# ramanathanlab/distllm

Hardware: NVIDIA H100
Metric: embedded chunks/sec @512-tok (higher is better)
Workload: dtype bf16

## Files before the change

### distllm_b200/csrc/b2e_api.cu

```cuda
#include "../../include/b2e.h"
#include "../../include/b2e_debug.h"

#include <cuda.h>
#include <cuda_runtime.h>

#include <cstdarg>
#include <cstdio>
#include <cstdlib>
#include <cstring>
#include <string>
#include <utility>
#include <vector>

#include "attention.cuh"
#include "binsearch.cuh"
#include "common.cuh"
#include "gemm.cuh"
#include "mistral_ops.cuh"
#include "pack.cuh"
#include "rowops.cuh"
#include "topk.cuh"
#include "topk_tc.cuh"

using namespace b2e;

#ifdef B2E_STORAGE_BF16
#define B2E_TMAP_DTYPE CU_TENSOR_MAP_DATA_TYPE_BFLOAT16
constexpr int kStorageDtype = B2E_DTYPE_BF16;
#else
#define B2E_TMAP_DTYPE CU_TENSOR_MAP_DATA_TYPE_FLOAT16
constexpr int kStorageDtype = B2E_DTYPE_F16;
#endif

namespace {

thread_local std::string g_err;

int fail(int code, const char* fmt, ...) {
  char buf[512];
  va_list ap;
  va_start(ap, fmt);
  vsnprintf(buf, sizeof buf, fmt, ap);
  va_end(ap);
  g_err = buf;
  return code;
}

#define CUDA_TRY(expr)                                                                    \
  do {                                                                                    \
    cudaError_t e_ = (expr);                                                              \
    if (e_ != cudaSuccess)                                                                \
      return fail(B2E_ERR_CUDA, "%s failed: %s (%s:%d)", #expr, cudaGetErrorString(e_),   \
                  __FILE__, __LINE__);                                                    \
  } while (0)

typedef CUresult (*EncodeTiledFn)(CUtensorMap*, CUtensorMapDataType, cuuint32_t, void*,
                                  const cuuint64_t*, const cuuint64_t*, const cuuint32_t*,
                                  const cuuint32_t*, CUtensorMapInterleave, CUtensorMapSwizzle,
                                  CUtensorMapL2promotion, CUtensorMapFloatOOBfill);

EncodeTiledFn get_encode_fn() {
  static EncodeTiledFn fn = nullptr;
  if (fn) return fn;
  void* p = nullptr;
  cudaDriverEntryPointQueryResult q;
  if (cudaGetDriverEntryPoint("cuTensorMapEncodeTiled", &p, cudaEnableDefault, &q) != cudaSuccess ||
      q != cudaDriverEntryPointSuccess)
    return nullptr;
  fn = reinterpret_cast<EncodeTiledFn>(p);
  return fn;
}

int make_tmap_h16(CUtensorMap* tm, const void* base, uint64_t rows, uint64_t cols,
                   uint32_t box_rows, uint32_t box_cols = 64) {
  EncodeTiledFn fn = get_encode_fn();
  if (!fn) return fail(B2E_ERR_CUDA, "cuTensorMapEncodeTiled entry point unavailable");
  cuuint64_t dims[2] = {cols, rows};
  cuuint64_t strides[1] = {cols * 2};
  cuuint32_t box[2] = {box_cols, box_rows};
  cuuint32_t estr[2] = {1, 1};
  CUresult r = fn(tm, B2E_TMAP_DTYPE, 2, const_cast<void*>(base), dims, strides,
                  box, estr, CU_TENSOR_MAP_INTERLEAVE_NONE,
                  box_cols == 64 ? CU_TENSOR_MAP_SWIZZLE_128B : CU_TENSOR_MAP_SWIZZLE_64B,
                  CU_TENSOR_MAP_L2_PROMOTION_L2_256B, CU_TENSOR_MAP_FLOAT_OOB_FILL_NONE);
  if (r != CUDA_SUCCESS)
    return fail(B2E_ERR_CUDA, "cuTensorMapEncodeTiled(rows=%llu, cols=%llu, box_rows=%u) -> %d",
                (unsigned long long)rows, (unsigned long long)cols, box_rows, (int)r);
  return B2E_OK;
}

int make_tmap_f32(CUtensorMap* tm, const void* base, uint64_t rows, uint64_t cols, uint32_t box_rows) {
  EncodeTiledFn fn = get_encode_fn();
  if (!fn) return fail(B2E_ERR_CUDA, "cuTensorMapEncodeTiled entry point unavailable");
  cuuint64_t dims[2] = {cols, rows};
  cuuint64_t strides[1] = {cols * 4};
  cuuint32_t box[2] = {32, box_rows};
  cuuint32_t estr[2] = {1, 1};
  CUresult r = fn(tm, CU_TENSOR_MAP_DATA_TYPE_FLOAT32, 2, const_cast<void*>(base), dims, strides, box, estr,
                  CU_TENSOR_MAP_INTERLEAVE_NONE, CU_TENSOR_MAP_SWIZZLE_128B, CU_TENSOR_MAP_L2_PROMOTION_L2_256B,
                  CU_TENSOR_MAP_FLOAT_OOB_FILL_NONE);
  if (r != CUDA_SUCCESS)
    return fail(B2E_ERR_CUDA, "cuTensorMapEncodeTiled f32(rows=%llu, cols=%llu, box_rows=%u) -> %d",
                (unsigned long long)rows, (unsigned long long)cols, box_rows, (int)r);
  return B2E_OK;
}

struct DeviceInfo {
  int sms = 0;
  int cc_major = 0;
  bool ok = false;
};

int device_info(int device, DeviceInfo* info) {
  int n = 0;
  if (cudaGetDeviceCount(&n) != cudaSuccess || n == 0) {
    cudaGetLastError();
    return fail(B2E_ERR_NO_DEVICE, "no CUDA device visible; libb2e has no CPU fallback");
  }
  if (device < 0 || device >= n) return fail(B2E_ERR_INVALID, "device %d out of range", device);
  cudaDeviceProp p;
  CUDA_TRY(cudaGetDeviceProperties(&p, device));
  if (p.major != 9 || p.minor != 0)
    return fail(B2E_ERR_NO_DEVICE, "device %d is sm_%d%d; libb2e is built for sm_90a only", device,
                p.major, p.minor);
  info->sms = p.multiProcessorCount;
  info->cc_major = p.major;
  info->ok = true;
  return B2E_OK;
}

int current_device_info(DeviceInfo* info) {
  int dev = 0;
  if (cudaGetDevice(&dev) != cudaSuccess) {
    cudaGetLastError();
    return fail(B2E_ERR_NO_DEVICE, "no CUDA device visible; libb2e has no CPU fallback");
  }
  static DeviceInfo cache[64];
  if (dev < 64 && cache[dev].ok) {
    *info = cache[dev];
    return B2E_OK;
  }
  int rc = device_info(dev, info);
  if (rc == B2E_OK && dev < 64) cache[dev] = *info;
  return rc;
}

template <typename Kern>
int ensure_smem_attr(Kern kern, int bytes) {
  static std::vector<std::pair<const void*, int>> done;
  int dev = 0;
  CUDA_TRY(cudaGetDevice(&dev));
  const void* key = reinterpret_cast<const void*>(kern);
  for (const auto& d : done)
    if (d.first == key && d.second == dev) return B2E_OK;
  CUDA_TRY(cudaFuncSetAttribute(kern, cudaFuncAttributeMaxDynamicSharedMemorySize, bytes));
  done.emplace_back(key, dev);
  return B2E_OK;
}

int check_gemm_shape(int M, int N, int K) {
  if (M <= 0 || N <= 0 || K <= 0) return fail(B2E_ERR_INVALID, "gemm: empty shape %dx%dx%d", M, N, K);
  if (N % 128 != 0) return fail(B2E_ERR_INVALID, "gemm: N=%d must be a multiple of 128", N);
  if (K % 64 != 0) return fail(B2E_ERR_INVALID, "gemm: K=%d must be a multiple of 64", K);
  return B2E_OK;
}

bool g_gemm_profiling = false;

template <int EPI>
int launch_gemm_epi(const CUtensorMap& ta, const CUtensorMap& tb, void* out, const float* bias,
                    const h16* resid, int M, int N, int K, cudaStream_t st, const int* m_dev) {
  auto kern = gemm_h16_wgmma_kernel<EPI>;
  if constexpr (EPI == EPI_BIAS)
    if (g_gemm_profiling) kern = gemm_h16_wgmma_kernel<EPI, true>;
  int rc = ensure_smem_attr(kern, GEMM_SMEM_BYTES);
  if (rc) return rc;
  DeviceInfo dev;
  if ((rc = current_device_info(&dev))) return rc;
  const long long tiles = (long long)(N / GEMM_BN) * ((M + GEMM_BM - 1) / GEMM_BM);
  if (tiles > 0x7fffffffLL) return fail(B2E_ERR_INVALID, "gemm: %lld output tiles exceed one grid", tiles);
  CUtensorMap tm_out;
  if ((rc = make_tmap_h16(&tm_out, out, M, epi_is_glu(EPI) ? N / 2 : N, GEMM_BM))) return rc;
  const unsigned grid = (unsigned)(tiles < dev.sms ? tiles : dev.sms);
  kern<<<grid, GEMM_THREADS, GEMM_SMEM_BYTES, st>>>(ta, tb, tm_out, static_cast<h16*>(out), bias, resid, M, N, K,
                                                    m_dev);
  CUDA_TRY(cudaGetLastError());
  return B2E_OK;
}

int launch_gemm(const CUtensorMap& ta, const CUtensorMap& tb, void* out, const float* bias,
                const void* resid, int M, int N, int K, int epi, cudaStream_t st, const int* m_dev = nullptr) {
  const h16* r = static_cast<const h16*>(resid);
  switch (epi) {
    case B2E_EPI_BIAS: return launch_gemm_epi<EPI_BIAS>(ta, tb, out, bias, r, M, N, K, st, m_dev);
    case B2E_EPI_BIAS_GELU: return launch_gemm_epi<EPI_BIAS_GELU>(ta, tb, out, bias, r, M, N, K, st, m_dev);
    case B2E_EPI_BIAS_RESID: return launch_gemm_epi<EPI_BIAS_RESID>(ta, tb, out, bias, r, M, N, K, st, m_dev);
    case B2E_EPI_SWIGLU: return launch_gemm_epi<EPI_SWIGLU>(ta, tb, out, bias, r, M, N, K, st, m_dev);
    case B2E_EPI_GEGLU: return launch_gemm_epi<EPI_GEGLU>(ta, tb, out, bias, r, M, N, K, st, m_dev);
  }
  return fail(B2E_ERR_INVALID, "unknown epilogue %d", epi);
}

struct AttnScratch {
  float* bias = nullptr;
  int* kv_chunks = nullptr;
  int* plain_chunks = nullptr;
  size_t cap_bias = 0, cap_b = 0;
  uint64_t gen = 0;
  int device = -1;
  int ensure(int B, int S_pad) {
    int dev = 0;
    CUDA_TRY(cudaGetDevice(&dev));
    if (dev != device) {
      release();
      device = dev;
      ++gen;
    }
    if ((size_t)B * S_pad > cap_bias || (size_t)B > cap_b) ++gen;
    if ((size_t)B * S_pad > cap_bias) {
      cudaFree(bias);
      bias = nullptr;
      cap_bias = 0;
      CUDA_TRY(cudaMalloc(&bias, sizeof(float) * (size_t)B * S_pad));
      cap_bias = (size_t)B * S_pad;
    }
    if ((size_t)B > cap_b) {
      cudaFree(kv_chunks); cudaFree(plain_chunks);
      kv_chunks = plain_chunks = nullptr;
      cap_b = 0;
      CUDA_TRY(cudaMalloc(&kv_chunks, sizeof(int) * B));
      CUDA_TRY(cudaMalloc(&plain_chunks, sizeof(int) * B));
      cap_b = B;
    }
    return B2E_OK;
  }
  void release() {
    cudaFree(bias); cudaFree(kv_chunks); cudaFree(plain_chunks);
    bias = nullptr; kv_chunks = plain_chunks = nullptr; cap_bias = cap_b = 0;
  }
};

inline int attn_s_pad(int S) { return (S + AT_KC - 1) / AT_KC * AT_KC; }

int attention_prepare(AttnScratch& sc, const int64_t* mask, int B, int S, cudaStream_t st) {
  int rc;
  const int S_pad = attn_s_pad(S);
  if ((rc = sc.ensure(B, S_pad))) return rc;
  attn_prep_kernel<<<(B + 7) / 8, 256, 0, st>>>(mask, sc.bias, sc.kv_chunks, sc.plain_chunks, B, S, S_pad);
  CUDA_TRY(cudaGetLastError());
  return B2E_OK;
}

struct SeqLayout {
  const int* cu = nullptr;
  const int* len = nullptr;
  const int* t_real = nullptr;
  const int* tok_src = nullptr;
};

template <int D, int MODE, int V>
int launch_attention_kernel(const CUtensorMap& tm, const AttnScratch& sc, void* ctx, int B, int S, int heads,
                            int kv_heads, int window, cudaStream_t st, const SeqLayout& lay) {
  using Cfg = AtCfg<D, V>;
  auto kern = attention_kernel<D, MODE, V>;
  int rc = ensure_smem_attr(kern, Cfg::SMEM_BYTES);
  if (rc) return rc;
  CUtensorMap tm_ctx = {};
  if ((V & 128) && (rc = make_tmap_h16(&tm_ctx, ctx, (uint64_t)B * S, (uint64_t)heads * D, 64, Cfg::COLS))) return rc;
  const float scale_log2e = 1.4426950408889634f / sqrtf(static_cast<float>(D));
  const long long ctas = (long long)heads * B * ((S + Cfg::QT - 1) / Cfg::QT);
  if (ctas > 0x7fffffffLL)
    return fail(B2E_ERR_INVALID, "attention: %lld CTAs (heads=%d B=%d S=%d) exceed one grid", ctas, heads, B, S);
  kern<<<(unsigned)ctas, Cfg::THREADS, Cfg::SMEM_BYTES, st>>>(tm, tm_ctx, sc.bias, sc.kv_chunks, sc.plain_chunks, B, S,
                                                    attn_s_pad(S), heads, kv_heads, window, scale_log2e, lay.cu,
                                                    lay.len, static_cast<h16*>(ctx));
  CUDA_TRY(cudaGetLastError());
  return B2E_OK;
}

constexpr int AT_DEFAULT_VARIANT = 193;
int g_att3_variant = -1;
inline int att3_variant() {
  if (g_att3_variant < 0) {
    const char* e = getenv("B2E_ATT3");
    g_att3_variant = e ? atoi(e) : AT_DEFAULT_VARIANT;
  }
  return g_att3_variant;
}

int launch_attention(const CUtensorMap& tkv, const AttnScratch& sc, void* ctx, int B, int S, int heads,
                     cudaStream_t st, int window = 0, const SeqLayout& lay = SeqLayout()) {
  const int v = att3_variant();
#define B2E_ATT(MODE, V) launch_attention_kernel<64, MODE, V>(tkv, sc, ctx, B, S, heads, heads, window, st, lay)
  if (window > 0) {
    switch (v & 192) {
      case 0: return B2E_ATT(1, 0);
      case 64: return B2E_ATT(1, 64);
      case 128: return B2E_ATT(1, 128);
      case 192: return B2E_ATT(1, 192);
    }
    return fail(B2E_ERR_INVALID, "windowed attention: variant %d has no instantiation (bits 6-7 of the variant pick "
                "0, 64, 128 or 192)", v);
  }
  switch (v) {
    case 0: return B2E_ATT(0, 0);
    case 1: return B2E_ATT(0, 1);
    case 5: return B2E_ATT(0, 5);
    case 64: return B2E_ATT(0, 64);
    case 65: return B2E_ATT(0, 65);
    case 69: return B2E_ATT(0, 69);
    case 193: return B2E_ATT(0, 193);
    case 261: return B2E_ATT(0, 261);
    case 321: return B2E_ATT(0, 321);
  }
#undef B2E_ATT
  return fail(B2E_ERR_INVALID, "attention variant %d is not instantiated (0,1,5,64,65,69,193,261,321)", v);
}

int launch_attention_causal_d128(const void* qkv, AttnScratch& sc, void* ctx, int B, int S, int heads,
                                 int kv_heads, int window, cudaStream_t st, const SeqLayout& lay = SeqLayout()) {
  CUtensorMap tm;
  const int rc = make_tmap_h16(&tm, qkv, (uint64_t)B * S, (uint64_t)(heads + 2 * kv_heads) * 128, AT_KC);
  if (rc) return rc;
  return launch_attention_kernel<128, 2, 0>(tm, sc, ctx, B, S, heads, kv_heads, window, st, lay);
}

constexpr int AT_D32_VARIANT = 1;

int launch_attention_bidir(const CUtensorMap& tqkv, const AttnScratch& sc, void* ctx, int B, int S, int heads,
                           int head_dim, cudaStream_t st, const SeqLayout& lay = SeqLayout()) {
  if (head_dim == 32)
    return launch_attention_kernel<32, 0, AT_D32_VARIANT>(tqkv, sc, ctx, B, S, heads, heads, 0, st, lay);
  return launch_attention(tqkv, sc, ctx, B, S, heads, st, 0, lay);
}

#define DISPATCH_H(H, CALL)                                         \
  switch (H) {                                                      \
    case 256: { constexpr int HW = 256; CALL; break; }              \
    case 384: { constexpr int HW = 384; CALL; break; }              \
    case 512: { constexpr int HW = 512; CALL; break; }              \
    case 640: { constexpr int HW = 640; CALL; break; }              \
    case 768: { constexpr int HW = 768; CALL; break; }              \
    case 1024: { constexpr int HW = 1024; CALL; break; }            \
    case 1280: { constexpr int HW = 1280; CALL; break; }            \
    case 2048: { constexpr int HW = 2048; CALL; break; }            \
    case 2560: { constexpr int HW = 2560; CALL; break; }            \
    case 4096: { constexpr int HW = 4096; CALL; break; }            \
    default: return fail(B2E_ERR_INVALID, "hidden size %d not supported (need 256*{1,2,3,4,5,8,10,16}, 384 or 640)", (H)); \
  }

inline int row_blocks(int rows) { return (rows + ROW_WARPS - 1) / ROW_WARPS; }

int check_h(int H) {
  if (H == 384 || H == 640) return B2E_OK;
  if (H % 256 != 0) return fail(B2E_ERR_INVALID, "hidden size %d must be a multiple of 256, or 384 or 640", H);
  switch (H / 256) {
    case 1: case 2: case 3: case 4: case 5: case 8: case 10: case 16: return B2E_OK;
  }
  return fail(B2E_ERR_UNSUPPORTED, "hidden size %d not supported (built: 256 x {1,2,3,4,5,8,10,16}, 384, 640)", H);
}

struct PoolScratch {
  int* seq_len = nullptr;
  int* kill = nullptr;
  int* idx = nullptr;
  float* w = nullptr;
  float* count = nullptr;
  float* part = nullptr;
  size_t cap_b = 0, cap_s = 0, cap_bs = 0, cap_part = 0;
  int device = -1;
  uint64_t gen = 0;

  int ensure(int B, int S, size_t part_elems) {
    int dev = 0;
    CUDA_TRY(cudaGetDevice(&dev));
    if (dev != device) {
      release();
      device = dev;
      ++gen;
    }
    if ((size_t)B > cap_b || (size_t)S > cap_s || (size_t)B * S > cap_bs || part_elems > cap_part) ++gen;
    if ((size_t)B > cap_b) {
      cudaFree(seq_len); cudaFree(idx); cudaFree(count);
      seq_len = idx = nullptr;
      count = nullptr;
      cap_b = 0;
      CUDA_TRY(cudaMalloc(&seq_len, sizeof(int) * B));
      CUDA_TRY(cudaMalloc(&idx, sizeof(int) * B));
      CUDA_TRY(cudaMalloc(&count, sizeof(float) * B));
      cap_b = B;
    }
    if ((size_t)S > cap_s) {
      cudaFree(kill);
      kill = nullptr;
      cap_s = 0;
      CUDA_TRY(cudaMalloc(&kill, sizeof(int) * S));
      cap_s = S;
    }
    if ((size_t)B * S > cap_bs) {
      cudaFree(w);
      w = nullptr;
      cap_bs = 0;
      CUDA_TRY(cudaMalloc(&w, sizeof(float) * (size_t)B * S));
      cap_bs = (size_t)B * S;
    }
    if (part_elems > cap_part) {
      cudaFree(part);
      part = nullptr;
      cap_part = 0;
      CUDA_TRY(cudaMalloc(&part, sizeof(float) * part_elems));
      cap_part = part_elems;
    }
    return B2E_OK;
  }
  void release() {
    cudaFree(seq_len); cudaFree(kill); cudaFree(idx); cudaFree(w); cudaFree(count); cudaFree(part);
    seq_len = kill = idx = nullptr; w = count = part = nullptr;
    cap_b = cap_s = cap_bs = cap_part = 0;
  }
};

inline int pool_nsplit(int S) {
  int n = (S + 63) / 64;
  return n < 1 ? 1 : (n > 16 ? 16 : n);
}

int launch_pool_weights(PoolScratch& ps, int64_t* mask, int B, int S, int pool_kind, int mutate,
                        cudaStream_t st) {
  seq_len_kernel<<<(B + 7) / 8, 256, 0, st>>>(mask, ps.seq_len, B, S);
  CUDA_TRY(cudaMemsetAsync(ps.kill, 0, sizeof(int) * S, st));
  kill_columns_kernel<<<(B + 255) / 256, 256, 0, st>>>(ps.seq_len, ps.kill, B, S);
  pool_weights_kernel<<<(B + 7) / 8, 256, 0, st>>>(mask, ps.seq_len, ps.kill, ps.w, ps.count, B, S,
                                                    pool_kind == B2E_POOL_MEAN_REF ? 1 : 0, mutate);
  CUDA_TRY(cudaGetLastError());
  return B2E_OK;
}

int launch_finalize(PoolScratch& ps, float* out, int B, int H, int nsplit, int l2, int round_mode,
                    cudaStream_t st) {
  pool_finalize_kernel<<<B, 256, (H + 32) * sizeof(float), st>>>(ps.part, ps.count, out, H, nsplit,
                                                                 l2, round_mode);
  CUDA_TRY(cudaGetLastError());
  return B2E_OK;
}

struct DeviceGuard {
  int prev = -1;
  DeviceGuard() {
    if (cudaGetDevice(&prev) != cudaSuccess) {
      cudaGetLastError();
      prev = -1;
    }
  }
  ~DeviceGuard() {
    if (prev >= 0) cudaSetDevice(prev);
  }
};

thread_local PoolScratch g_pool_scratch;
thread_local AttnScratch g_attn_scratch;

}

struct B2EEncoder {
  B2EModelDesc desc;
  int full_layers = 0;
  std::vector<const void*> w;
  int device = 0;
  int sms = 0;
  size_t cap_tokens = 0;
  h16 *hidden = nullptr, *qkv = nullptr, *ctx = nullptr, *tmp = nullptr, *ffn = nullptr;
  PoolScratch pool;
  AttnScratch attn;
  int *pk_len_raw = nullptr, *pk_ok = nullptr, *pk_len = nullptr, *pk_cu = nullptr, *pk_treal = nullptr,
// ... 1338 lines not shown
```

### distllm_b200/csrc/common.cuh

```cuda
#pragma once

#include <cuda.h>
#include <cuda_bf16.h>
#include <cuda_fp16.h>
#include <cuda_runtime.h>
#include <stdint.h>

namespace b2e {

using bf16 = __nv_bfloat16;
#ifdef B2E_STORAGE_BF16
using h16 = __nv_bfloat16;
#else
using h16 = __half;
#endif

__device__ __forceinline__ uint32_t smem_u32(const void* p) {
  return static_cast<uint32_t>(__cvta_generic_to_shared(p));
}

__device__ __forceinline__ uint32_t lane_id() { return threadIdx.x & 31u; }

__device__ __forceinline__ bool elect_one() {
  uint32_t pred = 0;
  asm volatile(
      "{\n\t"
      ".reg .pred p;\n\t"
      "elect.sync _|p, 0xffffffff;\n\t"
      "selp.u32 %0, 1, 0, p;\n\t"
      "}\n"
      : "=r"(pred));
  return pred != 0;
}

__device__ __forceinline__ void mbar_init(uint32_t bar, uint32_t count) {
  asm volatile("mbarrier.init.shared::cta.b64 [%0], %1;" ::"r"(bar), "r"(count) : "memory");
}
__device__ __forceinline__ void mbar_fence_init() {
  asm volatile("fence.mbarrier_init.release.cluster;" ::: "memory");
}
__device__ __forceinline__ void mbar_expect_tx(uint32_t bar, uint32_t bytes) {
  asm volatile("mbarrier.arrive.expect_tx.shared::cta.b64 _, [%0], %1;" ::"r"(bar), "r"(bytes)
               : "memory");
}
__device__ __forceinline__ void mbar_arrive(uint32_t bar) {
  asm volatile("mbarrier.arrive.shared::cta.b64 _, [%0];" ::"r"(bar) : "memory");
}
__device__ __forceinline__ bool mbar_try_wait(uint32_t bar, uint32_t parity) {
  uint32_t ok;
  asm volatile(
      "{\n\t"
      ".reg .pred p;\n\t"
      "mbarrier.try_wait.parity.shared::cta.b64 p, [%1], %2;\n\t"
      "selp.u32 %0, 1, 0, p;\n\t"
      "}\n"
      : "=r"(ok)
      : "r"(bar), "r"(parity)
      : "memory");
  return ok != 0;
}
__device__ __forceinline__ bool mbar_test(uint32_t bar, uint32_t parity) {
  uint32_t ok;
  asm volatile(
      "{\n\t"
      ".reg .pred p;\n\t"
      "mbarrier.test_wait.parity.shared::cta.b64 p, [%1], %2;\n\t"
      "selp.u32 %0, 1, 0, p;\n\t"
      "}\n"
      : "=r"(ok)
      : "r"(bar), "r"(parity)
      : "memory");
  return ok != 0;
}
__device__ __forceinline__ void mbar_wait(uint32_t bar, uint32_t parity) {
  while (!mbar_try_wait(bar, parity)) {
  }
}

__device__ __forceinline__ void mbar_wait_parked(uint32_t bar, uint32_t parity) {
  asm volatile(
      "{\n\t"
      ".reg .pred p;\n\t"
      "B2E_WAIT:\n\t"
      "mbarrier.try_wait.parity.shared::cta.b64 p, [%0], %1, %2;\n\t"
      "@p bra B2E_DONE;\n\t"
      "bra B2E_WAIT;\n\t"
      "B2E_DONE:\n\t"
      "}\n" ::"r"(bar),
      "r"(parity), "r"(0x989680)
      : "memory");
}

__device__ __forceinline__ void fence_proxy_async_smem() {
  asm volatile("fence.proxy.async.shared::cta;" ::: "memory");
}
__device__ __forceinline__ void st_shared_u32(uint32_t addr, uint32_t v) {
  asm volatile("st.shared.b32 [%0], %1;" ::"r"(addr), "r"(v) : "memory");
}

__device__ __forceinline__ void named_bar_sync(int id, int threads) {
  asm volatile("bar.sync %0, %1;" ::"r"(id), "r"(threads) : "memory");
}
__device__ __forceinline__ void named_bar_arrive(int id, int threads) {
  asm volatile("bar.arrive %0, %1;" ::"r"(id), "r"(threads) : "memory");
}

__device__ __forceinline__ void tma_prefetch_desc(const CUtensorMap* m) {
  asm volatile("prefetch.tensormap [%0];" ::"l"(m) : "memory");
}
__device__ __forceinline__ void tma_load_2d(uint32_t dst, const CUtensorMap* m, uint32_t bar,
                                            int c0, int c1) {
  asm volatile(
      "cp.async.bulk.tensor.2d.shared::cluster.global.mbarrier::complete_tx::bytes"
      " [%0], [%1, {%3, %4}], [%2];"
      ::"r"(dst), "l"(m), "r"(bar), "r"(c0), "r"(c1)
      : "memory");
}
__device__ __forceinline__ void bulk_load_1d(uint32_t dst, const void* src, uint32_t bytes,
                                             uint32_t bar) {
  asm volatile(
      "cp.async.bulk.shared::cluster.global.mbarrier::complete_tx::bytes [%0], [%1], %2, [%3];"
      ::"r"(dst), "l"(src), "r"(bytes), "r"(bar)
      : "memory");
}
__device__ __forceinline__ void tma_prefetch_l2_2d(const CUtensorMap* m, int c0, int c1) {
  asm volatile("cp.async.bulk.prefetch.tensor.2d.L2.global.tile [%0, {%1, %2}];" ::"l"(m), "r"(c0),
               "r"(c1)
               : "memory");
}
__device__ __forceinline__ void tma_store_2d(const CUtensorMap* m, uint32_t src, int c0, int c1) {
  asm volatile("cp.async.bulk.tensor.2d.global.shared::cta.bulk_group [%0, {%2, %3}], [%1];"
               ::"l"(m), "r"(src), "r"(c0), "r"(c1)
               : "memory");
}
__device__ __forceinline__ void tma_store_3d(const CUtensorMap* m, uint32_t src, int c0, int c1,
                                             int c2) {
  asm volatile("cp.async.bulk.tensor.3d.global.shared::cta.bulk_group [%0, {%2, %3, %4}], [%1];"
               ::"l"(m), "r"(src), "r"(c0), "r"(c1), "r"(c2)
               : "memory");
}
__device__ __forceinline__ void tma_store_commit() {
  asm volatile("cp.async.bulk.commit_group;" ::: "memory");
}
__device__ __forceinline__ void tma_store_wait_all() {
  asm volatile("cp.async.bulk.wait_group 0;" ::: "memory");
}
template <int N>
__device__ __forceinline__ void tma_store_wait_read() {
  asm volatile("cp.async.bulk.wait_group.read %0;" ::"n"(N) : "memory");
}

__device__ __forceinline__ void wgmma_fence() { asm volatile("wgmma.fence.sync.aligned;" ::: "memory"); }
__device__ __forceinline__ void wgmma_commit() { asm volatile("wgmma.commit_group.sync.aligned;" ::: "memory"); }
template <int N>
__device__ __forceinline__ void wgmma_wait() {
  asm volatile("wgmma.wait_group.sync.aligned %0;" ::"n"(N) : "memory");
}
template <int R>
__device__ __forceinline__ void reg_fence(float (&d)[R]) {
#pragma unroll
  for (int i = 0; i < R; ++i) asm volatile("" : "+f"(d[i])::"memory");
}

__device__ __forceinline__ uint64_t make_smem_desc_sw128(uint32_t saddr) {
  uint64_t d = 0;
  d |= static_cast<uint64_t>((saddr >> 4) & 0x3FFFu);
  d |= static_cast<uint64_t>(1u) << 16;
  d |= static_cast<uint64_t>(1024u >> 4) << 32;
  d |= static_cast<uint64_t>(1) << 62;
  return d;
}

__device__ __forceinline__ uint64_t make_smem_desc_sw64(uint32_t saddr) {
  uint64_t d = 0;
  d |= static_cast<uint64_t>((saddr >> 4) & 0x3FFFu);
  d |= static_cast<uint64_t>(1u) << 16;
  d |= static_cast<uint64_t>(512u >> 4) << 32;
  d |= static_cast<uint64_t>(2) << 62;
  return d;
}

#ifdef B2E_STORAGE_BF16
#define B2E_WGMMA_AB "bf16.bf16"
#else
#define B2E_WGMMA_AB "f16.f16"
#endif

template <int TRANS_B>
__device__ __forceinline__ void wgmma_64x64_ss(float (&d)[32], uint64_t a, uint64_t b, int accumulate) {
  asm volatile(
      "{\n.reg .pred p;\nsetp.ne.b32 p, %34, 0;\n"
      "wgmma.mma_async.sync.aligned.m64n64k16.f32." B2E_WGMMA_AB " "
      "{%0,%1,%2,%3,%4,%5,%6,%7,%8,%9,%10,%11,%12,%13,%14,%15,"
      "%16,%17,%18,%19,%20,%21,%22,%23,%24,%25,%26,%27,%28,%29,%30,%31}, %32, %33, p, 1, 1, 0, %35;\n}\n"
      : "+f"(d[0]), "+f"(d[1]), "+f"(d[2]), "+f"(d[3]), "+f"(d[4]), "+f"(d[5]), "+f"(d[6]), "+f"(d[7]),
        "+f"(d[8]), "+f"(d[9]), "+f"(d[10]), "+f"(d[11]), "+f"(d[12]), "+f"(d[13]), "+f"(d[14]), "+f"(d[15]),
        "+f"(d[16]), "+f"(d[17]), "+f"(d[18]), "+f"(d[19]), "+f"(d[20]), "+f"(d[21]), "+f"(d[22]), "+f"(d[23]),
        "+f"(d[24]), "+f"(d[25]), "+f"(d[26]), "+f"(d[27]), "+f"(d[28]), "+f"(d[29]), "+f"(d[30]), "+f"(d[31])
      : "l"(a), "l"(b), "r"(accumulate), "n"(TRANS_B));
}

__device__ __forceinline__ void wgmma_64x64_rs_tb(float (&d)[32], const uint32_t (&a)[4], uint64_t b) {
  asm volatile(
      "{\n.reg .pred p;\nsetp.eq.u32 p, 1, 1;\n"
      "wgmma.mma_async.sync.aligned.m64n64k16.f32." B2E_WGMMA_AB " "
      "{%0,%1,%2,%3,%4,%5,%6,%7,%8,%9,%10,%11,%12,%13,%14,%15,"
      "%16,%17,%18,%19,%20,%21,%22,%23,%24,%25,%26,%27,%28,%29,%30,%31}, {%32,%33,%34,%35}, %36, p, 1, 1, 1;\n}\n"
      : "+f"(d[0]), "+f"(d[1]), "+f"(d[2]), "+f"(d[3]), "+f"(d[4]), "+f"(d[5]), "+f"(d[6]), "+f"(d[7]),
        "+f"(d[8]), "+f"(d[9]), "+f"(d[10]), "+f"(d[11]), "+f"(d[12]), "+f"(d[13]), "+f"(d[14]), "+f"(d[15]),
        "+f"(d[16]), "+f"(d[17]), "+f"(d[18]), "+f"(d[19]), "+f"(d[20]), "+f"(d[21]), "+f"(d[22]), "+f"(d[23]),
        "+f"(d[24]), "+f"(d[25]), "+f"(d[26]), "+f"(d[27]), "+f"(d[28]), "+f"(d[29]), "+f"(d[30]), "+f"(d[31])
      : "r"(a[0]), "r"(a[1]), "r"(a[2]), "r"(a[3]), "l"(b));
}

__device__ __forceinline__ void wgmma_64x32_rs_tb(float (&d)[16], const uint32_t (&a)[4], uint64_t b) {
  asm volatile(
      "{\n.reg .pred p;\nsetp.eq.u32 p, 1, 1;\n"
      "wgmma.mma_async.sync.aligned.m64n32k16.f32." B2E_WGMMA_AB " "
      "{%0,%1,%2,%3,%4,%5,%6,%7,%8,%9,%10,%11,%12,%13,%14,%15}, {%16,%17,%18,%19}, %20, p, 1, 1, 1;\n}\n"
      : "+f"(d[0]), "+f"(d[1]), "+f"(d[2]), "+f"(d[3]), "+f"(d[4]), "+f"(d[5]), "+f"(d[6]), "+f"(d[7]),
        "+f"(d[8]), "+f"(d[9]), "+f"(d[10]), "+f"(d[11]), "+f"(d[12]), "+f"(d[13]), "+f"(d[14]), "+f"(d[15])
      : "r"(a[0]), "r"(a[1]), "r"(a[2]), "r"(a[3]), "l"(b));
}

__device__ __forceinline__ void wgmma_64x128_ss(float (&d)[64], uint64_t a, uint64_t b, int accumulate) {
  asm volatile(
      "{\n.reg .pred p;\nsetp.ne.b32 p, %66, 0;\n"
      "wgmma.mma_async.sync.aligned.m64n128k16.f32." B2E_WGMMA_AB " "
      "{%0,%1,%2,%3,%4,%5,%6,%7,%8,%9,%10,%11,%12,%13,%14,%15,"
      "%16,%17,%18,%19,%20,%21,%22,%23,%24,%25,%26,%27,%28,%29,%30,%31,"
      "%32,%33,%34,%35,%36,%37,%38,%39,%40,%41,%42,%43,%44,%45,%46,%47,"
      "%48,%49,%50,%51,%52,%53,%54,%55,%56,%57,%58,%59,%60,%61,%62,%63}, %64, %65, p, 1, 1, 0, 0;\n}\n"
      : "+f"(d[0]), "+f"(d[1]), "+f"(d[2]), "+f"(d[3]), "+f"(d[4]), "+f"(d[5]), "+f"(d[6]), "+f"(d[7]),
        "+f"(d[8]), "+f"(d[9]), "+f"(d[10]), "+f"(d[11]), "+f"(d[12]), "+f"(d[13]), "+f"(d[14]), "+f"(d[15]),
        "+f"(d[16]), "+f"(d[17]), "+f"(d[18]), "+f"(d[19]), "+f"(d[20]), "+f"(d[21]), "+f"(d[22]), "+f"(d[23]),
        "+f"(d[24]), "+f"(d[25]), "+f"(d[26]), "+f"(d[27]), "+f"(d[28]), "+f"(d[29]), "+f"(d[30]), "+f"(d[31]),
        "+f"(d[32]), "+f"(d[33]), "+f"(d[34]), "+f"(d[35]), "+f"(d[36]), "+f"(d[37]), "+f"(d[38]), "+f"(d[39]),
        "+f"(d[40]), "+f"(d[41]), "+f"(d[42]), "+f"(d[43]), "+f"(d[44]), "+f"(d[45]), "+f"(d[46]), "+f"(d[47]),
        "+f"(d[48]), "+f"(d[49]), "+f"(d[50]), "+f"(d[51]), "+f"(d[52]), "+f"(d[53]), "+f"(d[54]), "+f"(d[55]),
        "+f"(d[56]), "+f"(d[57]), "+f"(d[58]), "+f"(d[59]), "+f"(d[60]), "+f"(d[61]), "+f"(d[62]), "+f"(d[63])
      : "l"(a), "l"(b), "r"(accumulate));
}

__device__ __forceinline__ void wgmma_64x16_tf32(float (&d)[8], uint64_t a, uint64_t b, int accumulate) {
  asm volatile(
      "{\n.reg .pred p;\nsetp.ne.b32 p, %10, 0;\n"
      "wgmma.mma_async.sync.aligned.m64n16k8.f32.tf32.tf32 {%0,%1,%2,%3,%4,%5,%6,%7}, %8, %9, p, 1, 1;\n}\n"
      : "+f"(d[0]), "+f"(d[1]), "+f"(d[2]), "+f"(d[3]), "+f"(d[4]), "+f"(d[5]), "+f"(d[6]), "+f"(d[7])
      : "l"(a), "l"(b), "r"(accumulate));
}


__device__ __forceinline__ uint32_t pack_h16x2(float lo, float hi) {
  uint32_t r;
#ifdef B2E_STORAGE_BF16
  asm("cvt.rn.bf16x2.f32 %0, %1, %2;" : "=r"(r) : "f"(hi), "f"(lo));
#else
  asm("cvt.rn.satfinite.f16x2.f32 %0, %1, %2;" : "=r"(r) : "f"(hi), "f"(lo));
#endif
  return r;
}
__device__ __forceinline__ float2 unpack_h16x2(uint32_t u) {
#ifdef B2E_STORAGE_BF16
  __nv_bfloat162 v = *reinterpret_cast<__nv_bfloat162*>(&u);
  return __bfloat1622float2(v);
#else
  __half2 v = *reinterpret_cast<__half2*>(&u);
  return __half22float2(v);
#endif
}
__device__ __forceinline__ float2 unpack_bf16x2(uint32_t u) {
  __nv_bfloat162 v = *reinterpret_cast<__nv_bfloat162*>(&u);
  return __bfloat1622float2(v);
}
__device__ __forceinline__ h16 to_h16(float x) {
#ifdef B2E_STORAGE_BF16
  return __float2bfloat16_rn(x);
#else
  h16 r;
  asm("cvt.rn.satfinite.f16.f32 %0, %1;" : "=h"(*reinterpret_cast<unsigned short*>(&r)) : "f"(x));
  return r;
#endif
}
__device__ __forceinline__ float from_h16(h16 x) {
#ifdef B2E_STORAGE_BF16
  return __bfloat162float(x);
#else
  return __half2float(x);
#endif
}
__device__ __forceinline__ float fast_exp2(float x) {
  float y;
  asm("ex2.approx.ftz.f32 %0, %1;" : "=f"(y) : "f"(x));
  return y;
}
__device__ __forceinline__ float warp_sum(float v) {
#pragma unroll
  for (int o = 16; o > 0; o >>= 1) v += __shfl_xor_sync(0xffffffffu, v, o);
  return v;
}
__device__ __forceinline__ float warp_max(float v) {
#pragma unroll
  for (int o = 16; o > 0; o >>= 1) v = fmaxf(v, __shfl_xor_sync(0xffffffffu, v, o));
  return v;
}

}
```

### distllm_b200/csrc/gemm.cuh

```cuda
#pragma once

#include "common.cuh"

namespace b2e {

enum GemmEpi : int { EPI_BIAS = 0, EPI_BIAS_GELU = 1, EPI_BIAS_RESID = 2, EPI_SWIGLU = 3, EPI_GEGLU = 4 };
__host__ __device__ constexpr bool epi_is_glu(int epi) { return epi == EPI_SWIGLU || epi == EPI_GEGLU; }

constexpr int GEMM_BM = 128;
constexpr int GEMM_BN = 128;
constexpr int GEMM_BK = 64;
constexpr int GEMM_STAGES = 5;
constexpr int GEMM_THREADS = 384;
constexpr int GEMM_PRODUCER_REGS = 40, GEMM_CONSUMER_REGS = 232;
constexpr int GEMM_A_BYTES = GEMM_BM * GEMM_BK * 2;
constexpr int GEMM_STAGE_BYTES = GEMM_A_BYTES + GEMM_BN * GEMM_BK * 2;
constexpr int GEMM_OUT_BOX = GEMM_BM * 64 * 2;
constexpr int GEMM_OUT_OFFSET = GEMM_STAGES * GEMM_STAGE_BYTES;
constexpr int GEMM_BAR_OFFSET = GEMM_OUT_OFFSET + 2 * 2 * GEMM_OUT_BOX;
constexpr int GEMM_SMEM_BYTES = GEMM_BAR_OFFSET + 16 * GEMM_STAGES + 1024;
static_assert(GEMM_SMEM_BYTES <= 232448, "shared memory of one SM");
constexpr int GEMM_BAR_TURN = 1, GEMM_BAR_STAGE = 3;

__device__ __forceinline__ float gelu_erf_fast(float x) {
  const float xc = fminf(fmaxf(x, -5.65685f), 5.65685f);
  const float v = xc * xc;
  float q = fmaf(v, -1.35688221e-05f, -1.95764464e-04f);
  q = fmaf(v, q, 3.65498251e-02f);
  q = fmaf(v, q, 7.97818838e-01f);
  float t;
  asm("tanh.approx.f32 %0, %1;" : "=f"(t) : "f"(xc * q));
  const float h = 0.5f * x;
  return fmaf(h, t, h);
}

__device__ __forceinline__ float gelu_erf(float x) {
  const float ax = fabsf(x);
  float t;
  asm("rcp.approx.ftz.f32 %0, %1;" : "=f"(t) : "f"(fmaf(0.3275911f * 0.70710678f, ax, 1.0f)));
  float p = fmaf(t, 1.061405429f, -1.453152027f);
  p = fmaf(t, p, 1.421413741f);
  p = fmaf(t, p, -0.284496736f);
  p = fmaf(t, p, 0.254829592f);
  p *= t;
  const float e = fast_exp2(ax * ax * (-0.5f * 1.4426950408889634f));
  return fmaxf(x, 0.0f) - 0.5f * ax * p * e;
}

__device__ __forceinline__ float silu(float x) {
  float r;
  asm("rcp.approx.ftz.f32 %0, %1;" : "=f"(r) : "f"(1.0f + fast_exp2(-1.4426950408889634f * x)));
  return x * r;
}


__device__ long long* g_gemm_clock = nullptr;

struct GemmTiles {
  int first, stride, count, n_tiles;
};
__device__ __forceinline__ GemmTiles gemm_tiles(int M, int N) {
  const int n_tiles = N / GEMM_BN;
  const int tiles = n_tiles * ((M + GEMM_BM - 1) / GEMM_BM);
  const int first = static_cast<int>(blockIdx.x), stride = static_cast<int>(gridDim.x);
  return {first, stride, first < tiles ? (tiles - 1 - first) / stride + 1 : 0, n_tiles};
}

template <int EPI, bool TL = false>
__global__ void __launch_bounds__(GEMM_THREADS, 1)
gemm_h16_wgmma_kernel(const __grid_constant__ CUtensorMap tm_a,
                      const __grid_constant__ CUtensorMap tm_b,
                      const __grid_constant__ CUtensorMap tm_out,
                      h16* __restrict__ out, const float* __restrict__ bias, const h16* __restrict__ resid,
                      int M, int N, int K, const int* __restrict__ m_dev) {
  if (m_dev != nullptr) M = __ldg(m_dev);
  const GemmTiles tl = gemm_tiles(M, N);
  extern __shared__ uint8_t smem_raw[];
  const uint32_t sb = (smem_u32(smem_raw) + 1023u) & ~1023u;
  const uint32_t full_bar = sb + GEMM_BAR_OFFSET;
  const uint32_t empty_bar = full_bar + 8u * GEMM_STAGES;
  const int warp = threadIdx.x >> 5;
  const int kblocks = K / GEMM_BK;

  if (threadIdx.x == 0) {
    for (int s = 0; s < GEMM_STAGES; ++s) {
      mbar_init(full_bar + 8u * s, 1);
      mbar_init(empty_bar + 8u * s, 1);
    }
    mbar_fence_init();
  }
  __syncthreads();

  long long* clk = (TL && blockIdx.x == 0) ? g_gemm_clock : nullptr;
  if (warp >= 8) {
    asm volatile("setmaxnreg.dec.sync.aligned.u32 %0;" ::"n"(GEMM_PRODUCER_REGS));
    if (warp == 8 && elect_one()) {
      tma_prefetch_desc(&tm_a);
      tma_prefetch_desc(&tm_b);
      int stage = 0, n = 0;
      uint32_t phase = 0;
      for (int i = 0; i < tl.count; ++i) {
        const int tile = tl.first + i * tl.stride;
        const int m0 = (tile / tl.n_tiles) * GEMM_BM, n0 = (tile % tl.n_tiles) * GEMM_BN;
        for (int kb = 0; kb < kblocks; ++kb, ++n) {
          mbar_wait(empty_bar + 8u * stage, phase ^ 1u);
          const uint32_t dst = sb + stage * GEMM_STAGE_BYTES;
          const uint32_t fb = full_bar + 8u * stage;
          mbar_expect_tx(fb, GEMM_STAGE_BYTES);
          tma_load_2d(dst, &tm_a, fb, kb * GEMM_BK, m0);
          tma_load_2d(dst + GEMM_A_BYTES, &tm_b, fb, kb * GEMM_BK, n0);
          if (TL && clk != nullptr && n < 256) clk[n] = clock64();
          if (++stage == GEMM_STAGES) { stage = 0; phase ^= 1u; }
        }
      }
    }
    return;
  }

  asm volatile("setmaxnreg.inc.sync.aligned.u32 %0;" ::"n"(GEMM_CONSUMER_REGS));
  const int wg = warp >> 2;
  const int t = threadIdx.x & 127;
  const int quad = t & 3;
  const int r_lo = 16 * (t >> 5) + ((t & 31) >> 2);
  const uint32_t stg = sb + GEMM_OUT_OFFSET + wg * (2 * GEMM_OUT_BOX);
  int retired = 0;
  for (int i = wg; i < tl.count; i += 2) {
    const int tile = tl.first + i * tl.stride;
    const int m0 = (tile / tl.n_tiles) * GEMM_BM, n_blk = tile % tl.n_tiles;
    float acc[2][64];
#pragma unroll
    for (int x = 0; x < 64; ++x) acc[0][x] = acc[1][x] = 0.0f;
    if (i > 0) named_bar_sync(GEMM_BAR_TURN + wg, 256);
    const int it = i * kblocks;
    int stage = it % GEMM_STAGES;
    uint32_t phase = (it / GEMM_STAGES) & 1u;
    int prev = -1;
    for (int kb = 0; kb < kblocks; ++kb) {
      mbar_wait(full_bar + 8u * stage, phase);
      const uint32_t a_addr = sb + stage * GEMM_STAGE_BYTES;
      const uint64_t a0 = make_smem_desc_sw128(a_addr), a1 = make_smem_desc_sw128(a_addr + 64 * 128);
      const uint64_t b_desc = make_smem_desc_sw128(a_addr + GEMM_A_BYTES);
      reg_fence(acc[0]);
      reg_fence(acc[1]);
      wgmma_fence();
#pragma unroll
      for (int k = 0; k < GEMM_BK / 16; ++k) {
        wgmma_64x128_ss(acc[0], a0 + 2u * k, b_desc + 2u * k, (kb | k) != 0);
        wgmma_64x128_ss(acc[1], a1 + 2u * k, b_desc + 2u * k, (kb | k) != 0);
      }
      wgmma_commit();
      reg_fence(acc[0]);
      reg_fence(acc[1]);
      wgmma_wait<1>();
      reg_fence(acc[0]);
      reg_fence(acc[1]);
      if (prev >= 0 && t == 0) mbar_arrive(empty_bar + 8u * prev);
      if (TL && clk != nullptr && wg == 0 && t == 0 && retired < 256) clk[256 + retired] = clock64();
      ++retired;
      prev = stage;
      if (++stage == GEMM_STAGES) { stage = 0; phase ^= 1u; }
    }
    if (i + 1 < tl.count) named_bar_arrive(GEMM_BAR_TURN + (wg ^ 1), 256);
    wgmma_wait<0>();
    reg_fence(acc[0]);
    reg_fence(acc[1]);
    if (t == 0) mbar_arrive(empty_bar + 8u * prev);

    const bool staged = m0 + GEMM_BM <= M;
    if (staged) {
      if (t == 0) tma_store_wait_read<0>();
      named_bar_sync(GEMM_BAR_STAGE + wg, 128);
    }
    if constexpr (epi_is_glu(EPI)) {
      const int n_out = N / 2;
#pragma unroll
      for (int j = 0; j < 8; ++j)
#pragma unroll
        for (int h = 0; h < 2; ++h)
#pragma unroll
          for (int half = 0; half < 2; ++half) {
            const int r = 64 * h + r_lo + 8 * half;
            const float g0 = acc[h][4 * j + 2 * half], g1 = acc[h][4 * j + 2 * half + 1];
            const float u0 = acc[h][4 * (j + 8) + 2 * half], u1 = acc[h][4 * (j + 8) + 2 * half + 1];
            float v0, v1;
            if (EPI == EPI_GEGLU) {
              v0 = gelu_erf_fast(g0) * u0;
              v1 = gelu_erf_fast(g1) * u1;
            } else {
              v0 = silu(g0) * u0;
              v1 = silu(g1) * u1;
            }
            if (staged)
              st_shared_u32(stg + r * 128 + ((j ^ (r & 7)) << 4) + 4 * quad, pack_h16x2(v0, v1));
            else if (m0 + r < M)
              *reinterpret_cast<uint32_t*>(out + static_cast<size_t>(m0 + r) * n_out + n_blk * (GEMM_BN / 2) +
                                           8 * j + 2 * quad) = pack_h16x2(v0, v1);
          }
    } else {
      const int col0 = n_blk * GEMM_BN + 2 * quad;
#pragma unroll
      for (int j = 0; j < 16; ++j) {
        const float2 b = bias != nullptr ? __ldg(reinterpret_cast<const float2*>(bias + col0 + 8 * j))
                                         : make_float2(0.0f, 0.0f);
#pragma unroll
        for (int h = 0; h < 2; ++h)
#pragma unroll
          for (int half = 0; half < 2; ++half) {
            const int r = 64 * h + r_lo + 8 * half;
            if (!staged && m0 + r >= M) continue;
            float v0 = acc[h][4 * j + 2 * half], v1 = acc[h][4 * j + 2 * half + 1];
            if (bias != nullptr) {
              v0 += b.x;
              v1 += b.y;
            }
            if (EPI == EPI_BIAS_GELU) {
              v0 = gelu_erf_fast(v0);
              v1 = gelu_erf_fast(v1);
            }
            const size_t off = static_cast<size_t>(m0 + r) * N + col0 + 8 * j;
            if (EPI == EPI_BIAS_RESID) {
              const float2 rv = unpack_h16x2(*reinterpret_cast<const uint32_t*>(resid + off));
              v0 += rv.x;
              v1 += rv.y;
            }
            if (staged)
              st_shared_u32(stg + (j >> 3) * GEMM_OUT_BOX + r * 128 + (((j & 7) ^ (r & 7)) << 4) + 4 * quad,
                            pack_h16x2(v0, v1));
            else
              *reinterpret_cast<uint32_t*>(out + off) = pack_h16x2(v0, v1);
          }
      }
    }
    if (staged) {
      fence_proxy_async_smem();
      named_bar_sync(GEMM_BAR_STAGE + wg, 128);
      if (t == 0) {
        if constexpr (epi_is_glu(EPI)) {
          tma_store_2d(&tm_out, stg, n_blk * (GEMM_BN / 2), m0);
        } else {
          tma_store_2d(&tm_out, stg, n_blk * GEMM_BN, m0);
          tma_store_2d(&tm_out, stg + GEMM_OUT_BOX, n_blk * GEMM_BN + 64, m0);
        }
        tma_store_commit();
      }
    }
  }
  if (t == 0) tma_store_wait_all();
}

}
```

Baseline: 3163.

## Add cooperative 128x256 wgmma GEMM kernel for wide-N, deep-K shapes

Adds a persistent warp-specialized GEMM kernel in which two consumer warpgroups each compute a 64x256 slice using m64n256k16 wgmma. The tile is 128x256 with 4 pipeline stages and B loaded in two TMA halves. The launcher routes to this kernel when N is a multiple of 256 and K>=2048. The aim is higher operand reuse and fewer tiles per output for large projections like the MLP down-projection. In exchange it holds 128 fp32 accumulators per thread, which adds register pressure, and it has fewer tiles to spread across SMs.

After: 3261, median of 6. +3.1%, better.

```diff
diff --git a/distllm_b200/csrc/b2e_api.cu b/distllm_b200/csrc/b2e_api.cu
--- a/distllm_b200/csrc/b2e_api.cu
+++ b/distllm_b200/csrc/b2e_api.cu
@@ -168,8 +168,30 @@
 bool g_gemm_profiling = false;
 
 template <int EPI>
+int launch_gemm_coop(const CUtensorMap& ta, const CUtensorMap& tb, void* out, const float* bias,
+                     const h16* resid, int M, int N, int K, cudaStream_t st, const int* m_dev) {
+  auto kern = gemm_h16_coop_kernel<EPI>;
+  if constexpr (EPI == EPI_BIAS)
+    if (g_gemm_profiling) kern = gemm_h16_coop_kernel<EPI, true>;
+  int rc = ensure_smem_attr(kern, GEMMC_SMEM_BYTES);
+  if (rc) return rc;
+  DeviceInfo dev;
+  if ((rc = current_device_info(&dev))) return rc;
+  const long long tiles = (long long)(N / GEMMC_BN) * ((M + GEMM_BM - 1) / GEMM_BM);
+  if (tiles > 0x7fffffffLL) return fail(B2E_ERR_INVALID, "gemm: %lld output tiles exceed one grid", tiles);
+  CUtensorMap tm_out;
+  if ((rc = make_tmap_h16(&tm_out, out, M, epi_is_glu(EPI) ? N / 2 : N, 64))) return rc;
+  const unsigned grid = (unsigned)(tiles < dev.sms ? tiles : dev.sms);
+  kern<<<grid, GEMM_THREADS, GEMMC_SMEM_BYTES, st>>>(ta, tb, tm_out, static_cast<h16*>(out), bias, resid, M, N, K,
+                                                     m_dev);
+  CUDA_TRY(cudaGetLastError());
+  return B2E_OK;
+}
+
+template <int EPI>
 int launch_gemm_epi(const CUtensorMap& ta, const CUtensorMap& tb, void* out, const float* bias,
                     const h16* resid, int M, int N, int K, cudaStream_t st, const int* m_dev) {
+  if (N % GEMMC_BN == 0 && K >= 2048) return launch_gemm_coop<EPI>(ta, tb, out, bias, resid, M, N, K, st, m_dev);
   auto kern = gemm_h16_wgmma_kernel<EPI>;
   if constexpr (EPI == EPI_BIAS)
     if (g_gemm_profiling) kern = gemm_h16_wgmma_kernel<EPI, true>;
diff --git a/distllm_b200/csrc/common.cuh b/distllm_b200/csrc/common.cuh
--- a/distllm_b200/csrc/common.cuh
+++ b/distllm_b200/csrc/common.cuh
@@ -242,6 +242,39 @@
       : "l"(a), "l"(b), "r"(accumulate));
 }
 
+__device__ __forceinline__ void wgmma_64x256_ss(float (&d)[128], uint64_t a, uint64_t b, int accumulate) {
+  asm volatile(
+      "{\n.reg .pred p;\nsetp.ne.b32 p, %130, 0;\n"
+      "wgmma.mma_async.sync.aligned.m64n256k16.f32." B2E_WGMMA_AB " "
+      "{"
+      "%0,%1,%2,%3,%4,%5,%6,%7,%8,%9,%10,%11,%12,%13,%14,%15,"
+      "%16,%17,%18,%19,%20,%21,%22,%23,%24,%25,%26,%27,%28,%29,%30,%31,"
+      "%32,%33,%34,%35,%36,%37,%38,%39,%40,%41,%42,%43,%44,%45,%46,%47,"
+      "%48,%49,%50,%51,%52,%53,%54,%55,%56,%57,%58,%59,%60,%61,%62,%63,"
+      "%64,%65,%66,%67,%68,%69,%70,%71,%72,%73,%74,%75,%76,%77,%78,%79,"
+      "%80,%81,%82,%83,%84,%85,%86,%87,%88,%89,%90,%91,%92,%93,%94,%95,"
+      "%96,%97,%98,%99,%100,%101,%102,%103,%104,%105,%106,%107,%108,%109,%110,%111,"
+      "%112,%113,%114,%115,%116,%117,%118,%119,%120,%121,%122,%123,%124,%125,%126,%127"
+      "}, %128, %129, p, 1, 1, 0, 0;\n}\n"
+      : "+f"(d[0]), "+f"(d[1]), "+f"(d[2]), "+f"(d[3]), "+f"(d[4]), "+f"(d[5]), "+f"(d[6]), "+f"(d[7]),
+        "+f"(d[8]), "+f"(d[9]), "+f"(d[10]), "+f"(d[11]), "+f"(d[12]), "+f"(d[13]), "+f"(d[14]), "+f"(d[15]),
+        "+f"(d[16]), "+f"(d[17]), "+f"(d[18]), "+f"(d[19]), "+f"(d[20]), "+f"(d[21]), "+f"(d[22]), "+f"(d[23]),
+        "+f"(d[24]), "+f"(d[25]), "+f"(d[26]), "+f"(d[27]), "+f"(d[28]), "+f"(d[29]), "+f"(d[30]), "+f"(d[31]),
+        "+f"(d[32]), "+f"(d[33]), "+f"(d[34]), "+f"(d[35]), "+f"(d[36]), "+f"(d[37]), "+f"(d[38]), "+f"(d[39]),
+        "+f"(d[40]), "+f"(d[41]), "+f"(d[42]), "+f"(d[43]), "+f"(d[44]), "+f"(d[45]), "+f"(d[46]), "+f"(d[47]),
+        "+f"(d[48]), "+f"(d[49]), "+f"(d[50]), "+f"(d[51]), "+f"(d[52]), "+f"(d[53]), "+f"(d[54]), "+f"(d[55]),
+        "+f"(d[56]), "+f"(d[57]), "+f"(d[58]), "+f"(d[59]), "+f"(d[60]), "+f"(d[61]), "+f"(d[62]), "+f"(d[63]),
+        "+f"(d[64]), "+f"(d[65]), "+f"(d[66]), "+f"(d[67]), "+f"(d[68]), "+f"(d[69]), "+f"(d[70]), "+f"(d[71]),
+        "+f"(d[72]), "+f"(d[73]), "+f"(d[74]), "+f"(d[75]), "+f"(d[76]), "+f"(d[77]), "+f"(d[78]), "+f"(d[79]),
+        "+f"(d[80]), "+f"(d[81]), "+f"(d[82]), "+f"(d[83]), "+f"(d[84]), "+f"(d[85]), "+f"(d[86]), "+f"(d[87]),
+        "+f"(d[88]), "+f"(d[89]), "+f"(d[90]), "+f"(d[91]), "+f"(d[92]), "+f"(d[93]), "+f"(d[94]), "+f"(d[95]),
+        "+f"(d[96]), "+f"(d[97]), "+f"(d[98]), "+f"(d[99]), "+f"(d[100]), "+f"(d[101]), "+f"(d[102]), "+f"(d[103]),
+        "+f"(d[104]), "+f"(d[105]), "+f"(d[106]), "+f"(d[107]), "+f"(d[108]), "+f"(d[109]), "+f"(d[110]), "+f"(d[111]),
+        "+f"(d[112]), "+f"(d[113]), "+f"(d[114]), "+f"(d[115]), "+f"(d[116]), "+f"(d[117]), "+f"(d[118]), "+f"(d[119]),
+        "+f"(d[120]), "+f"(d[121]), "+f"(d[122]), "+f"(d[123]), "+f"(d[124]), "+f"(d[125]), "+f"(d[126]), "+f"(d[127])
+      : "l"(a), "l"(b), "r"(accumulate));
+}
+
 __device__ __forceinline__ void wgmma_64x16_tf32(float (&d)[8], uint64_t a, uint64_t b, int accumulate) {
   asm volatile(
       "{\n.reg .pred p;\nsetp.ne.b32 p, %10, 0;\n"
diff --git a/distllm_b200/csrc/gemm.cuh b/distllm_b200/csrc/gemm.cuh
--- a/distllm_b200/csrc/gemm.cuh
+++ b/distllm_b200/csrc/gemm.cuh
@@ -248,4 +248,204 @@
   if (t == 0) tma_store_wait_all();
 }
 
-}
+
+constexpr int GEMMC_BN = 256;
+constexpr int GEMMC_STAGES = 4;
+constexpr int GEMMC_W_HALF = GEMM_BN * GEMM_BK * 2;
+constexpr int GEMMC_STAGE_BYTES = GEMM_A_BYTES + 2 * GEMMC_W_HALF;
+constexpr int GEMMC_OUT_BOX = 64 * 64 * 2;
+constexpr int GEMMC_OUT_OFFSET = GEMMC_STAGES * GEMMC_STAGE_BYTES;
+constexpr int GEMMC_BAR_OFFSET = GEMMC_OUT_OFFSET + 2 * 2 * GEMMC_OUT_BOX;
+constexpr int GEMMC_SMEM_BYTES = GEMMC_BAR_OFFSET + 16 * GEMMC_STAGES + 1024;
+static_assert(GEMMC_SMEM_BYTES <= 232448, "shared memory of one SM");
+
+__device__ __forceinline__ GemmTiles gemm_tiles_256(int M, int N) {
+  const int n_tiles = N / GEMMC_BN;
+  const int tiles = n_tiles * ((M + GEMM_BM - 1) / GEMM_BM);
+  const int first = static_cast<int>(blockIdx.x), stride = static_cast<int>(gridDim.x);
+  return {first, stride, first < tiles ? (tiles - 1 - first) / stride + 1 : 0, n_tiles};
+}
+
+template <int EPI, bool TL = false>
+__global__ void __launch_bounds__(GEMM_THREADS, 1)
+gemm_h16_coop_kernel(const __grid_constant__ CUtensorMap tm_a,
+                     const __grid_constant__ CUtensorMap tm_b,
+                     const __grid_constant__ CUtensorMap tm_out,
+                     h16* __restrict__ out, const float* __restrict__ bias, const h16* __restrict__ resid,
+                     int M, int N, int K, const int* __restrict__ m_dev) {
+  if (m_dev != nullptr) M = __ldg(m_dev);
+  const GemmTiles tl = gemm_tiles_256(M, N);
+  extern __shared__ uint8_t smem_raw[];
+  const uint32_t sb = (smem_u32(smem_raw) + 1023u) & ~1023u;
+  const uint32_t full_bar = sb + GEMMC_BAR_OFFSET;
+  const uint32_t empty_bar = full_bar + 8u * GEMMC_STAGES;
+  const int warp = threadIdx.x >> 5;
+  const int kblocks = K / GEMM_BK;
+
+  if (threadIdx.x == 0) {
+    for (int s = 0; s < GEMMC_STAGES; ++s) {
+      mbar_init(full_bar + 8u * s, 1);
+      mbar_init(empty_bar + 8u * s, 2);
+    }
+    mbar_fence_init();
+  }
+  __syncthreads();
+
+  long long* clk = (TL && blockIdx.x == 0) ? g_gemm_clock : nullptr;
+  if (warp >= 8) {
+    asm volatile("setmaxnreg.dec.sync.aligned.u32 %0;" ::"n"(GEMM_PRODUCER_REGS));
+    if (warp == 8 && elect_one()) {
+      tma_prefetch_desc(&tm_a);
+      tma_prefetch_desc(&tm_b);
+      int stage = 0, n = 0;
+      uint32_t phase = 0;
+      for (int i = 0; i < tl.count; ++i) {
+        const int tile = tl.first + i * tl.stride;
+        const int m0 = (tile / tl.n_tiles) * GEMM_BM, n0 = (tile % tl.n_tiles) * GEMMC_BN;
+        for (int kb = 0; kb < kblocks; ++kb, ++n) {
+          mbar_wait(empty_bar + 8u * stage, phase ^ 1u);
+          const uint32_t dst = sb + stage * GEMMC_STAGE_BYTES;
+          const uint32_t fb = full_bar + 8u * stage;
+          mbar_expect_tx(fb, GEMMC_STAGE_BYTES);
+          tma_load_2d(dst, &tm_a, fb, kb * GEMM_BK, m0);
+          tma_load_2d(dst + GEMM_A_BYTES, &tm_b, fb, kb * GEMM_BK, n0);
+          tma_load_2d(dst + GEMM_A_BYTES + GEMMC_W_HALF, &tm_b, fb, kb * GEMM_BK, n0 + GEMM_BN);
+          if (TL && clk != nullptr && n < 256) clk[n] = clock64();
+          if (++stage == GEMMC_STAGES) { stage = 0; phase ^= 1u; }
+        }
+      }
+    }
+    return;
+  }
+
+  asm volatile("setmaxnreg.inc.sync.aligned.u32 %0;" ::"n"(GEMM_CONSUMER_REGS));
+  const int wg = warp >> 2;
+  const int t = threadIdx.x & 127;
+  const int quad = t & 3;
+  const int r_lo = 16 * (t >> 5) + ((t & 31) >> 2);
+  const uint32_t stg = sb + GEMMC_OUT_OFFSET + wg * (2 * GEMMC_OUT_BOX);
+  int stage = 0, retired = 0;
+  uint32_t phase = 0;
+  for (int i = 0; i < tl.count; ++i) {
+    const int tile = tl.first + i * tl.stride;
+    const int n_blk = tile % tl.n_tiles;
+    const int mr = (tile / tl.n_tiles) * GEMM_BM + 64 * wg;
+    float acc[128];
+#pragma unroll
+    for (int x = 0; x < 128; ++x) acc[x] = 0.0f;
+    int prev = -1;
+    for (int kb = 0; kb < kblocks; ++kb) {
+      mbar_wait(full_bar + 8u * stage, phase);
+      const uint32_t s_addr = sb + stage * GEMMC_STAGE_BYTES;
+      const uint64_t a_desc = make_smem_desc_sw128(s_addr + wg * (64 * 128));
+      const uint64_t b_desc = make_smem_desc_sw128(s_addr + GEMM_A_BYTES);
+      reg_fence(acc);
+      wgmma_fence();
+#pragma unroll
+      for (int k = 0; k < GEMM_BK / 16; ++k) wgmma_64x256_ss(acc, a_desc + 2u * k, b_desc + 2u * k, (kb | k) != 0);
+      wgmma_commit();
+      reg_fence(acc);
+      wgmma_wait<1>();
+      reg_fence(acc);
+      if (prev >= 0 && t == 0) mbar_arrive(empty_bar + 8u * prev);
+      if (TL && clk != nullptr && wg == 0 && t == 0 && retired < 256) clk[256 + retired] = clock64();
+      ++retired;
+      prev = stage;
+      if (++stage == GEMMC_STAGES) { stage = 0; phase ^= 1u; }
+    }
+    wgmma_wait<0>();
+    reg_fence(acc);
+    if (t == 0) mbar_arrive(empty_bar + 8u * prev);
+
+    const bool staged = mr + 64 <= M;
+    if constexpr (epi_is_glu(EPI)) {
+      const int n_out = N / 2;
+#pragma unroll
+      for (int s = 0; s < 2; ++s) {
+        if (staged) {
+          if (t == 0) tma_store_wait_read<1>();
+          named_bar_sync(GEMM_BAR_STAGE + wg, 128);
+        }
+#pragma unroll
+        for (int j = 0; j < 8; ++j)
+#pragma unroll
+          for (int half = 0; half < 2; ++half) {
+            const int r = r_lo + 8 * half;
+            const float g0 = acc[4 * (16 * s + j) + 2 * half], g1 = acc[4 * (16 * s + j) + 2 * half + 1];
+            const float u0 = acc[4 * (16 * s + j + 8) + 2 * half], u1 = acc[4 * (16 * s + j + 8) + 2 * half + 1];
+            float v0, v1;
+            if (EPI == EPI_GEGLU) {
+              v0 = gelu_erf_fast(g0) * u0;
+              v1 = gelu_erf_fast(g1) * u1;
+            } else {
+              v0 = silu(g0) * u0;
+              v1 = silu(g1) * u1;
+            }
+            if (staged)
+              st_shared_u32(stg + s * GEMMC_OUT_BOX + r * 128 + ((j ^ (r & 7)) << 4) + 4 * quad, pack_h16x2(v0, v1));
+            else if (mr + r < M)
+              *reinterpret_cast<uint32_t*>(out + static_cast<size_t>(mr + r) * n_out + n_blk * (GEMMC_BN / 2) +
+                                           64 * s + 8 * j + 2 * quad) = pack_h16x2(v0, v1);
+          }
+        if (staged) {
+          fence_proxy_async_smem();
+          named_bar_sync(GEMM_BAR_STAGE + wg, 128);
+          if (t == 0) {
+            tma_store_2d(&tm_out, stg + s * GEMMC_OUT_BOX, n_blk * (GEMMC_BN / 2) + 64 * s, mr);
+            tma_store_commit();
+          }
+        }
+      }
+    } else {
+#pragma unroll
+      for (int q = 0; q < 4; ++q) {
+        if (staged) {
+          if (t == 0) tma_store_wait_read<1>();
+          named_bar_sync(GEMM_BAR_STAGE + wg, 128);
+        }
+        const int col0 = n_blk * GEMMC_BN + 64 * q + 2 * quad;
+        const uint32_t box = stg + (q & 1) * GEMMC_OUT_BOX;
+#pragma unroll
+        for (int j = 0; j < 8; ++j) {
+          const float2 b = bias != nullptr ? __ldg(reinterpret_cast<const float2*>(bias + col0 + 8 * j))
+                                           : make_float2(0.0f, 0.0f);
+#pragma unroll
+          for (int half = 0; half < 2; ++half) {
+            const int r = r_lo + 8 * half;
+            if (!staged && mr + r >= M) continue;
+            float v0 = acc[4 * (8 * q + j) + 2 * half], v1 = acc[4 * (8 * q + j) + 2 * half + 1];
+            if (bias != nullptr) {
+              v0 += b.x;
+              v1 += b.y;
+            }
+            if (EPI == EPI_BIAS_GELU) {
+              v0 = gelu_erf_fast(v0);
+              v1 = gelu_erf_fast(v1);
+            }
+            const size_t off = static_cast<size_t>(mr + r) * N + col0 + 8 * j;
+            if (EPI == EPI_BIAS_RESID) {
+              const float2 rv = unpack_h16x2(*reinterpret_cast<const uint32_t*>(resid + off));
+              v0 += rv.x;
+              v1 += rv.y;
+            }
+            if (staged)
+              st_shared_u32(box + r * 128 + ((j ^ (r & 7)) << 4) + 4 * quad, pack_h16x2(v0, v1));
+            else
+              *reinterpret_cast<uint32_t*>(out + off) = pack_h16x2(v0, v1);
+          }
+        }
+        if (staged) {
+          fence_proxy_async_smem();
+          named_bar_sync(GEMM_BAR_STAGE + wg, 128);
+          if (t == 0) {
+            tma_store_2d(&tm_out, box, n_blk * GEMMC_BN + 64 * q, mr);
+            tma_store_commit();
+          }
+        }
+      }
+    }
+  }
+  if (t == 0) tma_store_wait_all();
+}
+
+}
```
